# RobotVisionHKA/LiFCal

Hardware: AMD Instinct MI355X
Metric: micro-image obs/sec through Jacobian+Schur at 1M obs (higher is better)
Workload: dtype f64; 1 GPU; metric_web: 334 frames, 24720 points, 999994 micro-image observations, window 10, config 0xf06 (2 radial + tangential, mlCenterAdj, Cauchy(0.5), refine poses+points); lens_selection=reference generator (lifcal_mla_project), obs_per_gpu=999994, n_reduced=2021, deterministic=False

## Files before the change

lifcal_amd/csrc/device_model.hpp:

```cpp
#pragma once
#include <hip/hip_runtime.h>

namespace lifcal {

#define LIFCAL_DEV __device__ __forceinline__

constexpr int NCMAX = 9;
constexpr int LENS_STRIDE = 16;
constexpr int FRAME_STRIDE = 16;

struct CamConsts {
  double fL, bL0, B, ifL;
  double craw[2];
  double sp[2], isp[2];
  double D, iD, e, zC0, gamma, beta;
  double de[3], dzC0[3], dgamma[3], dbeta[3];
  double a, da[3];
  double k[2], p[2];
  double chm[NCMAX];
  double loss_b, loss_c;
};

LIFCAL_DEV void cam_prepare(const double* cam, double spx, double spy, double scale, int n_radial, bool tangential,
                            unsigned fixed_mask, double loss_scale, bool fold, CamConsts& c) {
  double sg[3] = {1.0, 1.0, 1.0};
  double th[3];
  for (int i = 0; i < 3; ++i) { th[i] = cam[i]; if (fold && th[i] < 0.0) { th[i] = -th[i]; sg[i] = -1.0; } }
  c.fL = th[0]; c.bL0 = th[1]; c.B = th[2]; c.ifL = 1.0 / c.fL;
  double dcr[2];
  for (int i = 0; i < 2; ++i) {
    double v = (cam[3 + i] + 0.5) * scale - 0.5; dcr[i] = scale;
    if (fold && v < 0.0) { v = -v; dcr[i] = -scale; }
    c.craw[i] = v;
  }
  c.sp[0] = spx / scale; c.sp[1] = spy / scale; c.isp[0] = 1.0 / c.sp[0]; c.isp[1] = 1.0 / c.sp[1];
  const double D = c.fL - c.bL0, iD = 1.0 / D, iD2 = iD * iD;
  c.D = D; c.iD = iD;
  c.e = c.fL * iD; c.zC0 = c.fL * c.bL0 * iD; c.gamma = c.fL * c.B * iD; c.beta = c.B * iD;
  c.de[0] = -c.bL0 * iD2;          c.de[1] = c.fL * iD2;           c.de[2] = 0.0;
  c.dzC0[0] = -c.bL0 * c.bL0 * iD2; c.dzC0[1] = c.fL * c.fL * iD2;   c.dzC0[2] = 0.0;
  c.dgamma[0] = -c.B * c.bL0 * iD2; c.dgamma[1] = c.fL * c.B * iD2;  c.dgamma[2] = c.fL * iD;
  c.dbeta[0] = -c.B * iD2;          c.dbeta[1] = c.B * iD2;          c.dbeta[2] = iD;
  const double s = c.bL0 + c.B, is = 1.0 / s;
  c.a = c.bL0 * is; c.da[0] = 0.0; c.da[1] = c.B * is * is; c.da[2] = -c.bL0 * is * is;
  c.k[0] = n_radial > 0 ? cam[5] : 0.0; c.k[1] = n_radial > 1 ? cam[6] : 0.0;
  c.p[0] = tangential ? cam[5 + n_radial] : 0.0; c.p[1] = tangential ? cam[6 + n_radial] : 0.0;
  const int nc = 5 + n_radial + (tangential ? 2 : 0);
  for (int j = 0; j < NCMAX; ++j) {
    double ch = 1.0;
    if (j < 3) ch = sg[j]; else if (j < 5) ch = dcr[j - 3];
    const bool live = (j < nc) && !((fixed_mask >> j) & 1u);
    c.chm[j] = live ? ch : 0.0;
  }
  c.loss_b = loss_scale * loss_scale; c.loss_c = 1.0 / c.loss_b;
}

template <int NR, bool TAN>
struct Distortion {
  double dx, dy, A00, A01, A10, A11, r2, r4;
  LIFCAL_DEV void eval(double x, double y, const CamConsts& c, bool want_jac) {
    r2 = x * x + y * y; r4 = r2 * r2;
    double g = 0.0, gp = 0.0;
    if (NR >= 1) { g = c.k[0] * r2; gp = c.k[0]; }
    if (NR >= 2) { g += c.k[1] * r4; gp += 2.0 * c.k[1] * r2; }
    dx = x * g; dy = y * g;
    if (want_jac) { const double xy2 = 2.0 * x * y * gp; A00 = g + 2.0 * x * x * gp; A01 = xy2; A10 = xy2; A11 = g + 2.0 * y * y * gp; }
    if (TAN) {
      dx += c.p[0] * (r2 + 2.0 * x * x) + 2.0 * c.p[1] * x * y;
      dy += c.p[1] * (r2 + 2.0 * y * y) + 2.0 * c.p[0] * x * y;
      if (want_jac) {
        A00 += 6.0 * c.p[0] * x + 2.0 * c.p[1] * y; A01 += 2.0 * c.p[0] * y + 2.0 * c.p[1] * x;
        A10 += 2.0 * c.p[1] * x + 2.0 * c.p[0] * y; A11 += 6.0 * c.p[1] * y + 2.0 * c.p[0] * x;
      }
    }
  }
  LIFCAL_DEV void explicit_partial(int a, double x, double y, double& ex, double& ey) const {
    ex = 0.0; ey = 0.0;
    if (NR >= 1 && a == 2) { ex = x * r2; ey = y * r2; }
    if (NR >= 2 && a == 3) { ex = x * r4; ey = y * r4; }
    if (TAN && a == 2 + NR) { ex = r2 + 2.0 * x * x; ey = 2.0 * x * y; }
    if (TAN && a == 3 + NR) { ex = 2.0 * x * y; ey = r2 + 2.0 * y * y; }
  }
};

template <int NR, bool TAN>
LIFCAL_DEV void lens_eval(const CamConsts& c, double mx, double my, bool want_tangents, double* out) {
  constexpr int NA = 2 + NR + (TAN ? 2 : 0);
  const double cdx = (mx - c.craw[0]) * c.sp[0], cdy = (my - c.craw[1]) * c.sp[1];
// ... 391 lines not shown
```

lifcal_amd/csrc/kernels.hpp:

```cpp
#pragma once
#include <hip/hip_runtime.h>
#include <stdint.h>

#include <type_traits>

#include "../../include/lifcal_ba.h"
#include "device_model.hpp"
#include "lm_step.hpp"

namespace lifcal {

constexpr uint32_t DET_NF_MAX = 20;
constexpr int SCAL_COST = 0, SCAL_BAD_U = 1, SCAL_GMAX0 = 2, SCAL_N = 2 + 64;
constexpr int ST_GTD = 0, ST_DDD = 1, ST_STEP2 = 2, ST_X2 = 3, ST_CAND_COST = 4, ST_CHOL_FAIL = 5, ST_GMAX_RED = 6, ST_DIR = 7, ST_N = 8;

struct TileSet { uint32_t n_tiles; const uint32_t *tile_row0, *slot_pt, *slot_fr, *slot_cnt, *ell_lens; const double *ell_u, *ell_v; };

struct Dev {
  uint32_t F, P, Q, NA, bw, nc, n_tiles, n_slots, n_lenses, n_red, ld, M_local, n_owned;
  uint32_t n_radial, tangential, adj, robust, use_poses, use_points, rank, world;
  uint32_t fixed_mask;
  double spx, spy, scale, loss_scale;
  double lm_min, lm_max;
  double *cam, *views, *pts, *cam_c, *views_c, *pts_c;
// ... 238 lines not shown
      const uint32_t pr = 6 * fr;
      double* Sd = d.Sband + (size_t)fr * (d.bw + 1) * 36;
      const double fm = d.frame_live[fr] != 0 ? 1.0 : 0.0;
#pragma unroll
      for (int a = 0; a < 6; ++a)
#pragma unroll
        for (int bb = 0; bb <= a; ++bb) {
          double v;
          if (a < 3) v = GAG[a][bb]; else if (bb < 3) v = AG[a - 3][bb]; else v = Am[a - 3][bb - 3];
          v *= fm;
          atomicAdd(Sd + a * 6 + bb, v);
          if (a == bb) atomicAdd(d.hdiag + pr + a, v);
        }
#pragma unroll
      for (int a = 0; a < 3; ++a) {
        atomicAdd(d.gB + pr + a, fm * (Gr[0][a] * b[0] + Gr[1][a] * b[1] + Gr[2][a] * b[2]));
        atomicAdd(d.gB + pr + 3 + a, fm * b[a]);
      }
      const uint32_t camrow = 3 * d.Q;
#pragma unroll
      for (int j = 0; j < NC; ++j) {
        double* row = d.Sarrow + (size_t)(camrow + j) * d.ld + pr;
#pragma unroll
        for (int cidx = 0; cidx < 3; ++cidx) atomicAdd(row + cidx, fm * (C[0][j] * Gr[0][cidx] + C[1][j] * Gr[1][cidx] + C[2][j] * Gr[2][cidx]));
#pragma unroll
        for (int cidx = 0; cidx < 3; ++cidx) atomicAdd(row + 3 + cidx, fm * C[cidx][j]);
      }
      if (d.use_points) {
        double AR[3][3], U[3][3], gP[3], Wc[3][NC], Wv[3][6];
#pragma unroll
        for (int i = 0; i < 3; ++i)
#pragma unroll
          for (int j = 0; j < 3; ++j) AR[i][j] = Am[i][0] * R[j] + Am[i][1] * R[3 + j] + Am[i][2] * R[6 + j];
#pragma unroll
        for (int i = 0; i < 3; ++i) {
#pragma unroll
          for (int j = 0; j < 3; ++j) U[i][j] = R[i] * AR[0][j] + R[3 + i] * AR[1][j] + R[6 + i] * AR[2][j];
          gP[i] = R[i] * b[0] + R[3 + i] * b[1] + R[6 + i] * b[2];
#pragma unroll
          for (int j = 0; j < NC; ++j) Wc[i][j] = R[i] * C[0][j] + R[3 + i] * C[1][j] + R[6 + i] * C[2][j];
#pragma unroll
          for (int j = 0; j < 3; ++j) Wv[i][j] = R[i] * AG[0][j] + R[3 + i] * AG[1][j] + R[6 + i] * AG[2][j];
#pragma unroll
          for (int j = 0; j < 3; ++j) Wv[i][3 + j] = R[i] * Am[0][j] + R[3 + i] * Am[1][j] + R[6 + i] * Am[2][j];
        }
        double* acc = d.ptacc + (size_t)pt * 36;
        atomicAdd(acc + 0, U[0][0]); atomicAdd(acc + 1, U[1][0]); atomicAdd(acc + 2, U[2][0]);
        atomicAdd(acc + 3, U[1][1]); atomicAdd(acc + 4, U[2][1]); atomicAdd(acc + 5, U[2][2]);
#pragma unroll
        for (int i = 0; i < 3; ++i) atomicAdd(acc + 6 + i, gP[i]);
#pragma unroll
        for (int i = 0; i < 3; ++i)
#pragma unroll
          for (int j = 0; j < NC; ++j) atomicAdd(acc + 9 + i * NCMAX + j, Wc[i][j]);
        double* wv = d.Wv + (size_t)d.slot_gid[slot] * 18;
#pragma unroll
        for (int i = 0; i < 3; ++i)
#pragma unroll
          for (int j = 0; j < 6; ++j) wv[i * 6 + j] = fm * Wv[i][j];
      }
    }
  }
  const uint32_t camrow = 3 * d.Q, camcol = 6 * d.F + 3 * d.Q;
  {
    int t = 0;
#pragma unroll
    for (int i = 0; i < NC; ++i) {
#pragma unroll
      for (int j = 0; j <= i; ++j) {
        const double s = wave_sum(cc[t]);
        if (lane == (uint32_t)(t & 63)) { atomicAdd(d.Sarrow + (size_t)(camrow + i) * d.ld + camcol + j, s); if (i == j) atomicAdd(d.hdiag + camcol + i, s); }
        ++t;
      }
    }
#pragma unroll
    for (int i = 0; i < NC; ++i) { const double s = wave_sum(gc[i]); if (lane == (uint32_t)i) atomicAdd(d.gB + camcol + i, s); }
    const double s = wave_sum(cost);
    if (lane == 63) atomicAdd(d.scal + SCAL_COST, s);
  }
  if (d.deterministic) det_turn_pass(d, 0, wave);
}

LIFCAL_DEV double finalize_column(const Dev& d, uint32_t t, double radius) {
  const uint32_t F6 = 6 * d.F;
  bool live;
  if (t < F6) live = d.use_poses && d.frame_live[t / 6];
  else if (t < F6 + 3 * d.Q) live = true;
  else live = d.camc->chm[t - F6 - 3 * d.Q] != 0.0;
  double* diag = s_addr(d, t, t);
  double* rhs = d.Sarrow + (size_t)d.NA * d.ld;
  if (live) {
    const double s = d.sig_red[t];
    const double lam = fmin(fmax(d.hdiag[t] * s * s, d.lm_min), d.lm_max) / (lm_radius(d, radius) * s * s);
    d.lam_red[t] = lam;
    *diag += lam;
    rhs[t] = -d.gB[t] + d.rhsacc[t];
  } else {
    d.lam_red[t] = 0.0;
    *diag = 1.0;
    rhs[t] = 0.0;
  }
  return fabs(d.gB[t]);
}

}
#include "sweep2.hpp"
#include "sweep3.hpp"
#include "sweep4.hpp"
namespace lifcal {

__global__ void k_constraints(Dev d, int cost_only, const double* pts, double* cost_out) {
  for (uint32_t t = blockIdx.x * blockDim.x + threadIdx.x; t < d.M_local; t += gridDim.x * blockDim.x) {
  const uint32_t c = d.my_cons[t];
  const uint32_t pi = d.c_i[c], pj = d.c_j[c];
  const double* Pi = pts + 3 * (size_t)pi; const double* Pj = pts + 3 * (size_t)pj;
  const double dx = Pi[0] - Pj[0], dy = Pi[1] - Pj[1], dz = Pi[2] - Pj[2];
  const double n = sqrt(dx * dx + dy * dy + dz * dz);
  const double is = 1.0 / (d.c_sigma[c] + 0.000001);
  const double r = (n - d.c_dist[c]) * is;
  atomicAdd(cost_out, 0.5 * r * r);
  if (cost_only) continue;
  const double in = is / n;
  const double Ji[3] = {dx * in, dy * in, dz * in};
  const uint32_t F6 = 6 * d.F;
  const int32_t qi = d.promoted[pi], qj = d.promoted[pj];
  const uint32_t cj = F6 + 3 * (uint32_t)qj;
  for (int a = 0; a < 3; ++a) {
    for (int b = 0; b <= a; ++b) s_add(d, cj + a, cj + b, Ji[a] * Ji[b]);
    atomicAdd(d.hdiag + cj + a, Ji[a] * Ji[a]);
    atomicAdd(d.gB + cj + a, -Ji[a] * r);
  }
  if (qi < 0) {
    double* acc = d.ptacc + (size_t)pi * 36;
    atomicAdd(acc + 0, Ji[0] * Ji[0]); atomicAdd(acc + 1, Ji[1] * Ji[0]); atomicAdd(acc + 2, Ji[2] * Ji[0]);
    atomicAdd(acc + 3, Ji[1] * Ji[1]); atomicAdd(acc + 4, Ji[2] * Ji[1]); atomicAdd(acc + 5, Ji[2] * Ji[2]);
    for (int a = 0; a < 3; ++a) atomicAdd(acc + 6 + a, Ji[a] * r);
    double* wp = d.Wpart + (size_t)c * 9;
    for (int a = 0; a < 3; ++a) for (int b = 0; b < 3; ++b) wp[a * 3 + b] = -Ji[a] * Ji[b];
  } else {
    const uint32_t ci = F6 + 3 * (uint32_t)qi;
    for (int a = 0; a < 3; ++a) {
      for (int b = 0; b <= a; ++b) s_add(d, ci + a, ci + b, Ji[a] * Ji[b]);
      atomicAdd(d.hdiag + ci + a, Ji[a] * Ji[a]);
      atomicAdd(d.gB + ci + a, Ji[a] * r);
      for (int b = 0; b < 3; ++b) {
        const double v = -Ji[a] * Ji[b];
        if (ci > cj) atomicAdd(s_addr(d, ci + a, cj + b), v); else atomicAdd(s_addr(d, cj + b, ci + a), v);
      }
    }
  }
  }
}

__global__ void k_promote_diag(Dev d) {
  const uint32_t q = blockIdx.x * blockDim.x + threadIdx.x;
  if (q >= d.Q) return;
  const uint32_t p = d.promoted_ids[q];
  const double* acc = d.ptacc + (size_t)p * 36;
  const uint32_t col = 6 * d.F + 3 * q;
  atomicAdd(d.hdiag + col + 0, acc[0]); atomicAdd(d.hdiag + col + 1, acc[3]); atomicAdd(d.hdiag + col + 2, acc[5]);
}

__global__ void k_jacobi(Dev d, int enabled) {
  const uint32_t t = blockIdx.x * blockDim.x + threadIdx.x;
  if (t < d.n_red) d.sig_red[t] = enabled ? 1.0 / (1.0 + sqrt(d.hdiag[t])) : 1.0;
  if (t < d.P) {
    const double* acc = d.ptacc + (size_t)t * 36;
    d.sigP[3 * (size_t)t + 0] = enabled ? 1.0 / (1.0 + sqrt(acc[0])) : 1.0;
    d.sigP[3 * (size_t)t + 1] = enabled ? 1.0 / (1.0 + sqrt(acc[3])) : 1.0;
    d.sigP[3 * (size_t)t + 2] = enabled ? 1.0 / (1.0 + sqrt(acc[5])) : 1.0;
  }
}

struct WBlock { const double* W; uint32_t width, ldw, base; };

LIFCAL_DEV WBlock point_block(const Dev& d, uint32_t p, uint32_t bidx, uint32_t ns) {
  WBlock b;
  if (bidx == 0) { b.W = d.ptacc + (size_t)p * 36 + 9; b.width = d.nc; b.ldw = NCMAX; b.base = 6 * d.F + 3 * d.Q; }
  else if (bidx <= ns) { const uint32_t s = d.pt_slot0[p] + bidx - 1; b.W = d.Wv + (size_t)s * 18; b.width = 6; b.ldw = 6; b.base = 6 * d.gid_fr[s]; }
  else { const uint32_t c = d.pt_cons_list[d.pt_cons0[p] + (bidx - ns - 1)]; b.W = d.Wpart + (size_t)c * 9; b.width = 3; b.ldw = 3; b.base = 6 * d.F + 3 * (uint32_t)d.promoted[d.c_j[c]]; }
  return b;
}

__global__ __launch_bounds__(256) void k_schur(Dev d, double radius) {
  const uint32_t lane = threadIdx.x & 63u;
// ... 181 lines not shown
  double sum = 0.0;
  double* dst = nullptr;
  if (t < n1) {
    if (mode != 0) return;
    const uint32_t f = (uint32_t)(t / BS), r = (uint32_t)(t % BS), dd = r / 36, e = r % 36;
    if (dd > f || (dd == 0 && (e % 6) > (e / 6))) return;
    uint32_t b0, b1; covering(f - dd, f, b0, b1);
    for (uint32_t b = b0; b < b1; ++b) {
      const uint32_t flo = d.blk_flo[b], nf = d.blk_nf[b];
      if (f >= flo + nf) continue;
      const uint32_t lf = f - flo, lj = f - dd - flo;
      sum += d.det_slab[(size_t)b * d.det_stride + (size_t)(lf * (lf + 1) / 2 + lj) * 36 + e];
    }
    dst = d.Sband + t;
  } else if (t < n2) {
    if (mode != 0) return;
    const uint32_t q = (uint32_t)(t - n1), j = q / F6, col = q % F6, f = col / 6;
    uint32_t b0, b1; covering(f, f, b0, b1);
    for (uint32_t b = b0; b < b1; ++b) {
      const uint32_t flo = d.blk_flo[b], nf = d.blk_nf[b];
      if (f >= flo + nf) continue;
      sum += d.det_slab[(size_t)b * d.det_stride + lay.off_cp + (size_t)j * 6 * NFm + 6 * (f - flo) + col % 6];
    }
    dst = d.Sarrow + (size_t)(camrow + j) * d.ld + col;
  } else if (t < n3) {
    if (mode != 0) return;
    return;
  } else if (t < n4) {
    const uint32_t q = (uint32_t)(t - n3), w = q / F6, col = q % F6, f = col / 6;
    if (mode != 0 && w != 1) return;
    uint32_t b0, b1; covering(f, f, b0, b1);
    for (uint32_t b = b0; b < b1; ++b) {
      const uint32_t flo = d.blk_flo[b], nf = d.blk_nf[b];
      if (f >= flo + nf) continue;
      sum += d.det_slab[(size_t)b * d.det_stride + lay.off_vec + (size_t)w * vlen + 6 * (f - flo) + col % 6];
    }
    dst = (w == 0 ? d.gB : (w == 1 ? d.hdiag : d.rhsacc)) + col;
  } else if (t < n5) {
    return;
  } else {
    return;
  }
  *dst += sum;
}

__global__ __launch_bounds__(64) void k_det_reduce_all(Dev d, int mode) {
  const V2Lds lay(d.v2_nfmax, true, 256);
  const uint32_t NFm = lay.nfm, vlen = 6 * NFm + NCMAX + 3, NC = d.nc, NCC = NC * (NC + 1) / 2, nB = d.n_blocks;
  const uint32_t e = blockIdx.x, lane = threadIdx.x;
  const uint32_t camrow = 3 * d.Q, camcol = 6 * d.F + 3 * d.Q;
  uint32_t off; double* dst; bool is_max = false;
  if (e < NCC) {
    if (mode != 0) return;
    uint32_t i = 0; while ((i + 1) * (i + 2) / 2 <= e) ++i;
    off = lay.off_cc + e; dst = d.Sarrow + (size_t)(camrow + i) * d.ld + camcol + (e - i * (i + 1) / 2);
  } else if (e < NCC + 3 * NC) {
    const uint32_t q = e - NCC, w = q / NC, j = q % NC;
    if (mode != 0 && w != 1) return;
    off = lay.off_vec + w * vlen + 6 * NFm + j; dst = (w == 0 ? d.gB : (w == 1 ? d.hdiag : d.rhsacc)) + camcol + j;
  } else {
    if (mode != 0) return;
    const uint32_t q = e - NCC - 3 * NC;
    off = lay.off_fr + q; is_max = q == 2;
    dst = d.scal + (q == 0 ? SCAL_COST : (q == 1 ? SCAL_BAD_U : SCAL_GMAX0 + d.rank));
  }
  double v = 0.0;
  for (uint32_t b = lane; b < nB; b += 64) { const double x = d.det_slab[(size_t)b * d.det_stride + off]; v = is_max ? fmax(v, x) : v + x; }
#pragma unroll
  for (int m = 32; m >= 1; m >>= 1) { const double o = __shfl_xor(v, m, 64); v = is_max ? fmax(v, o) : v + o; }
  if (lane == 0) { if (is_max) *dst = fmax(*dst, v); else *dst += v; }
}

__global__ void k_det_sum(const double* slots, uint32_t n_wg, uint32_t K, double* dst) {
  const uint32_t k = threadIdx.x;
  if (k >= K) return;
  double s = 0.0;
  for (uint32_t g = 0; g < n_wg; ++g) s += slots[(size_t)g * K + k];
  dst[k] += s;
}

constexpr uint32_t FIN_ZERO_PER_WG = 256 * 4;
__global__ void k_finalize(Dev d, double radius, uint32_t n_fin, double* zero, uint32_t n_zero) {
  if (blockIdx.x >= n_fin) {
    const uint32_t n_threads = (gridDim.x - n_fin) * blockDim.x;
    for (uint32_t i = (blockIdx.x - n_fin) * blockDim.x + threadIdx.x; i < n_zero; i += n_threads) zero[i] = 0.0;
    return;
  }
  const uint32_t t = blockIdx.x * blockDim.x + threadIdx.x;
  if (t == 0) d.lm[LM_T0] = (double)__builtin_amdgcn_s_memrealtime();
  double g = 0.0;
  if (t < d.n_red) g = finalize_column(d, t, radius);
#pragma unroll
  for (int m = 32; m >= 1; m >>= 1) g = fmax(g, __shfl_xor(g, m, 64));
  if ((threadIdx.x & 63u) == 0) atomicMax((unsigned long long*)(d.step + ST_GMAX_RED), (unsigned long long)__double_as_longlong(g));
}

__global__ __launch_bounds__(1024) void k_band_chol(Dev d) {
  extern __shared__ __attribute__((aligned(16))) double smem[];
  double* Ld = smem; double* Li = smem + 36; double* failp = smem + 72;
  double* panel = d.panel_g ? d.panel_g : smem + 80;
  const uint32_t tid = threadIdx.x, nt = blockDim.x;
  const uint32_t F = d.F, bw = d.bw, NAx = d.NA + 1, ld = d.ld;
  if (tid == 0) *failp = 0.0;
  __syncthreads();
  for (uint32_t j = 0; j < F; ++j) {
    double* Sjj = d.Sband + (size_t)j * (bw + 1) * 36;
    if (tid == 0) {
      double L[6][6];
      for (int a = 0; a < 6; ++a) for (int b = 0; b <= a; ++b) L[a][b] = Sjj[a * 6 + b];
      bool ok = true;
      for (int c = 0; c < 6; ++c) {
        double dg = L[c][c];
        for (int k = 0; k < c; ++k) dg -= L[c][k] * L[c][k];
        if (!(dg > 0.0)) { ok = false; dg = 1.0; }
        dg = sqrt(dg); L[c][c] = dg;
        for (int r = c + 1; r < 6; ++r) { double s = L[r][c]; for (int k = 0; k < c; ++k) s -= L[r][k] * L[c][k]; L[r][c] = s / dg; }
      }
      if (!ok) *failp = 1.0;
      double I[6][6];
      for (int c = 0; c < 6; ++c) {
        for (int r = 0; r < 6; ++r) I[r][c] = 0.0;
        I[c][c] = 1.0 / L[c][c];
        for (int r = c + 1; r < 6; ++r) { double s = 0.0; for (int k = c; k < r; ++k) s -= L[r][k] * I[k][c]; I[r][c] = s / L[r][r]; }
      }
      for (int a = 0; a < 6; ++a) for (int b = 0; b < 6; ++b) { Ld[a * 6 + b] = (b <= a) ? L[a][b] : 0.0; Li[a * 6 + b] = (b <= a) ? I[a][b] : 0.0; }
      for (int a = 0; a < 6; ++a) for (int b = 0; b <= a; ++b) Sjj[a * 6 + b] = L[a][b];
      for (int k = 0; k < 36; ++k) d.Linv[(size_t)j * 36 + k] = Li[k];
    }
    __syncthreads();
    const uint32_t nbel = min(bw, F - 1 - j);
    const uint32_t nrows = 6 * nbel + NAx;
    for (uint32_t r = tid; r < nrows; r += nt) {
      double* src;
      if (r < 6 * nbel) { const uint32_t i = j + 1 + r / 6; src = d.Sband + ((size_t)i * (bw + 1) + (i - j)) * 36 + (r % 6) * 6; }
      else src = d.Sarrow + (size_t)(r - 6 * nbel) * ld + 6 * j;
      double x[6], y[6];
#pragma unroll
      for (int k = 0; k < 6; ++k) x[k] = src[k];
#pragma unroll
      for (int c = 0; c < 6; ++c) { double s = 0.0;
#pragma unroll
        for (int k = 0; k <= c; ++k) s += x[k] * Li[c * 6 + k];
        y[c] = s; }
#pragma unroll
      for (int k = 0; k < 6; ++k) { src[k] = y[k]; panel[(size_t)r * 6 + k] = y[k]; }
    }
    __syncthreads();
    const uint32_t nb6 = 6 * nbel;
    const uint64_t nband = (uint64_t)nb6 * (nb6 + 1) / 2;
    const uint64_t narrow = (uint64_t)NAx * nb6;
    const uint64_t naa = (uint64_t)NAx * (NAx + 1) / 2;
    for (uint64_t t = tid; t < nband + narrow + naa; t += nt) {
      uint32_t r, cidx; double* dst;
      if (t < nband) {
        r = (uint32_t)((sqrt(8.0 * (double)t + 1.0) - 1.0) * 0.5);
        while ((uint64_t)r * (r + 1) / 2 > t) --r;
        while ((uint64_t)(r + 1) * (r + 2) / 2 <= t) ++r;
        cidx = (uint32_t)(t - (uint64_t)r * (r + 1) / 2);
        const uint32_t bi = j + 1 + r / 6, bc = j + 1 + cidx / 6;
        dst = d.Sband + ((size_t)bi * (bw + 1) + (bi - bc)) * 36 + (r % 6) * 6 + (cidx % 6);
      } else if (t < nband + narrow) {
        const uint64_t u = t - nband; const uint32_t a = (uint32_t)(u / nb6); cidx = (uint32_t)(u % nb6); r = nb6 + a;
        dst = d.Sarrow + (size_t)a * ld + 6 * (j + 1) + cidx;
      } else {
        const uint64_t u = t - nband - narrow;
        uint32_t a = (uint32_t)((sqrt(8.0 * (double)u + 1.0) - 1.0) * 0.5);
        while ((uint64_t)a * (a + 1) / 2 > u) --a;
        while ((uint64_t)(a + 1) * (a + 2) / 2 <= u) ++a;
// ... 451 lines not shown
```

lifcal_amd/csrc/sweep3.hpp:

```cpp
#pragma once

namespace lifcal {

template <int NR, bool TAN, bool ADJ, int WR, class ET = double>
__global__ __launch_bounds__(128 * WR, 2) void k_sweep3(Dev d, double radius, int mode) {
  constexpr bool F32 = sizeof(ET) == 4;
  constexpr int NC = 5 + NR + (TAN ? 2 : 0);
  constexpr int NCC = NC * (NC + 1) / 2;
  constexpr int HV = 6 + 2 * NC + 2;
  constexpr uint32_t LP = 64u * WR;
  constexpr uint32_t NT = 2u * LP;
  static_assert(HV * LP <= V2Lds::zd_for(LP), "hand-off buffer must fit the Z matrix");
  if (radius < 0.0 && d.lm[LM_TERMINATION] != 0.0) return;
  extern __shared__ __attribute__((aligned(16))) double sm[];
  const V2Lds lay(d.v2_nfmax, true, LP);
  const uint32_t NFm = lay.nfm, vlen = 6 * NFm + NCMAX + 3;
  double* Spp = sm; double* Scp = sm + lay.off_cp; double* Scc = sm + lay.off_cc;
  double* vgB = sm + lay.off_vec; double* vhd = vgB + vlen; double* vrhs = vhd + vlen;
  double* Fr = sm + lay.off_fr;
  double* slab = sm + lay.off_slab;
  double* Zd = sm + lay.off_zd;
  double* misc = sm + lay.off_misc;
  uint32_t* pidl = (uint32_t*)(misc + MISC_DOUBLES);
  unsigned short* colinfo = (unsigned short*)(misc + MISC_DOUBLES + 32);
  uint32_t flip = 0;
#ifndef LIFCAL_NO_ROLE_FLIP
  if (WR == 2) flip = (__builtin_amdgcn_s_getreg(6 | (0 << 6) | (7 << 11)) != 0) ? LP : 0u;
#endif
  const uint32_t tid = threadIdx.x ^ flip, lane = tid & 63u, w = tid >> 6;
  const bool role_b = w >= (uint32_t)WR;
  const uint32_t wl = w & (uint32_t)(WR - 1);
  const uint32_t t256 = tid & (LP - 1u);
  const uint32_t b = blockIdx.x;
  const uint32_t flo = d.blk_flo[b], nf = d.blk_nf[b];
  const uint32_t ncol = 6 * nf + NC + 1, ncolp = (ncol + 15u) & ~15u;
  const uint32_t zs = ncolp + 2;
  const CamConsts c = *d.camc;
#ifdef LIFCAL_STAMPS
  unsigned long long st_acc[16] = {0, 0, 0, 0, 0, 0, 0, 0, 0, 0, 0, 0, 0, 0, 0, 0}, st_last = 0;
  if (tid == 0 || tid == LP) { asm volatile("s_memtime %0\n\ts_waitcnt lgkmcnt(0)" : "=s"(st_last) :: "memory"); }
#define STAMPB(i) do { if (tid == LP) { unsigned long long t_; asm volatile("s_memtime %0\n\ts_waitcnt lgkmcnt(0)" : "=s"(t_) :: "memory"); st_acc[i] += t_ - st_last; st_last = t_; } } while (0)
#else
#define STAMPB(i) do { } while (0)
#endif
  const uint32_t ps_begin = d.blk_pass0[b], ps_end = d.blk_pass0[b + 1];
  uint32_t nx_np = 0, nx_gid0 = 0, nx_si = 0, nx_pt = 0, nx_fp = 0, nx_gid = 0, nx_r[2] = {0, 0};
  uint32_t vz;
  asm volatile("v_mov_b32 %0, 0" : "=v"(vz));
  auto fetch_pass = [&](uint32_t q) {
    nx_np = d.pass_np[q + vz]; nx_gid0 = d.pass_gid0[q + vz];
    nx_si = d.v2_slot[(size_t)q * LP + t256]; nx_pt = d.v2f_pt[(size_t)q * LP + t256]; nx_gid = d.v2_gidx[(size_t)q * LP + t256];
    nx_r[0] = d.v2_tile_row0[q * WR + wl + vz]; nx_r[1] = d.v2_tile_row0[q * WR + wl + 1 + vz];
    nx_fp = d.v2_passpt[(size_t)q * 64 + (tid & 63u)];
  };
  if (ps_begin < ps_end) fetch_pass(ps_begin);
  { double2* z2 = reinterpret_cast<double2*>(sm); for (uint32_t i = tid; i < lay.off_slab / 2; i += NT) z2[i] = double2{0.0, 0.0}; }
  if (tid == 0 && (lay.off_slab & 1u)) sm[lay.off_slab - 1] = 0.0;
  if (tid < MISC_DOUBLES) misc[tid] = 0.0;
  for (uint32_t cI = tid; cI < ncolp; cI += NT)
    colinfo[cI] = (cI < 6 * nf) ? (unsigned short)(((cI / 6) << 8) | (cI % 6)) : (cI < ncol - 1 ? (unsigned short)(0x8000u | (cI - 6 * nf)) : (unsigned short)0xC000u);

  auto zero_slab = [&]() { for (uint32_t i = tid; i < lay.np_max * SLAB_STRIDE; i += NT) slab[i] = 0.0; };
  auto zero_zd = [&](uint32_t krows) { double2* z2 = reinterpret_cast<double2*>(Zd); for (uint32_t i = tid; i < (krows * zs) / 2; i += NT) z2[i] = double2{0.0, 0.0}; };
  auto z_phase = [&](uint32_t np) {
    const uint32_t nwc = ncol - 1;
    const uint32_t nth = NT / nwc > 0 ? NT / nwc : 1;
    const uint32_t gi = tid / nwc, cidx = tid - gi * nwc;
    if (gi < nth || nwc > NT) {
      for (uint32_t cc0 = cidx; cc0 < nwc; cc0 += (nwc > NT ? NT : nwc * nth)) {
#pragma unroll 4
        for (uint32_t lp = (nwc > NT ? 0 : gi); lp < np; lp += (nwc > NT ? 1 : nth)) {
          const double* acc = slab + lp * SLAB_STRIDE;
          double* z = Zd + (size_t)(3 * lp) * zs + cc0;
          const double w0 = z[0], w1 = z[zs], w2 = z[2 * zs];
          if (cc0 >= 6 * nf) {
            double* ga = d.ptacc + (size_t)pidl[lp] * 36 + 9 + (cc0 - 6 * nf);
            ga[0] = w0; ga[NCMAX] = w1; ga[2 * NCMAX] = w2;
          }
          z[0] = acc[0] * w0; z[zs] = acc[1] * w0 + acc[3] * w1; z[2 * zs] = acc[2] * w0 + acc[4] * w1 + acc[5] * w2;
        }
      }
    }
  };
  struct LaneGeom { double R[9], Y[3], Gr[3][3]; };
  auto lane_geom = [&](uint32_t fr, uint32_t pt, LaneGeom& q) {
    const double* ft = d.ft + (size_t)fr * FRAME_STRIDE;
    const double* P = d.pts + 3 * (size_t)pt;
#pragma unroll
    for (int k = 0; k < 9; ++k) q.R[k] = ft[k];
    const double P0 = P[0], P1 = P[1], P2 = P[2];
#pragma unroll
    for (int k = 0; k < 3; ++k) q.Y[k] = q.R[3 * k] * P0 + q.R[3 * k + 1] * P1 + q.R[3 * k + 2] * P2;
    const double c0 = ft[12], s0 = ft[13], n0 = q.R[2], n1 = q.R[5], n2 = q.R[8];
    q.Gr[0][0] = 0.0;     q.Gr[0][1] = c0 * q.Y[2] - s0 * q.Y[1]; q.Gr[0][2] = n1 * q.Y[2] - n2 * q.Y[1];
    q.Gr[1][0] = -q.Y[2]; q.Gr[1][1] = s0 * q.Y[0];               q.Gr[1][2] = n2 * q.Y[0] - n0 * q.Y[2];
    q.Gr[2][0] = q.Y[1];  q.Gr[2][1] = -c0 * q.Y[0];              q.Gr[2][2] = n0 * q.Y[1] - n1 * q.Y[0];
  };
  const uint32_t frs = NFm * lay.nrep;
  struct RunMask { double m1, m2, m4, m8; bool head; };
  auto run_masks = [&](uint32_t cnt, uint32_t lf) {
    const int key = cnt > 0 ? (int)lf : (int)(0x7F000000u + lane);
    RunMask r;
    r.m1 = __builtin_amdgcn_update_dpp(-1, key, 0x101, 0xf, 0xf, false) == key ? 1.0 : 0.0;
    r.m2 = __builtin_amdgcn_update_dpp(-1, key, 0x102, 0xf, 0xf, false) == key ? 1.0 : 0.0;
    r.m4 = __builtin_amdgcn_update_dpp(-1, key, 0x104, 0xf, 0xf, false) == key ? 1.0 : 0.0;
    r.m8 = __builtin_amdgcn_update_dpp(-1, key, 0x108, 0xf, 0xf, false) == key ? 1.0 : 0.0;
    r.head = cnt > 0 && __builtin_amdgcn_update_dpp(-1, key, 0x111, 0xf, 0xf, false) != key;
    return r;
  };
  auto run_sum = [](double v, const RunMask& r) {
    auto shl = [](double x, auto ctrl) {
      const int lo = __double2loint(x), hi = __double2hiint(x);
      return __hiloint2double(__builtin_amdgcn_update_dpp(0, hi, decltype(ctrl)::value, 0xf, 0xf, true),
                              __builtin_amdgcn_update_dpp(0, lo, decltype(ctrl)::value, 0xf, 0xf, true));
    };
    v = fma(shl(v, std::integral_constant<int, 0x101>{}), r.m1, v);
    v = fma(shl(v, std::integral_constant<int, 0x102>{}), r.m2, v);
    v = fma(shl(v, std::integral_constant<int, 0x104>{}), r.m4, v);
    v = fma(shl(v, std::integral_constant<int, 0x108>{}), r.m8, v);
    return v;
  };
  uint32_t* hw_written = (uint32_t*)(misc + 4) + wl;
  uint32_t* hw_read = (uint32_t*)(misc + 4) + 4 + wl;
  uint32_t* eval_done = (uint32_t*)(misc + 3);
  const bool det = d.deterministic != 0;
  uint32_t* turn = (uint32_t*)(misc + 8) + (role_b ? 1 : 0);
  uint32_t my_turn = wl;
  auto wait_for = [](uint32_t* flag, uint32_t need) {
    while (__hip_atomic_load(flag, __ATOMIC_ACQUIRE, __HIP_MEMORY_SCOPE_WORKGROUP) < need) __builtin_amdgcn_s_sleep(2);
  };
  auto publish = [](uint32_t* flag, uint32_t value) {
    asm volatile("s_waitcnt lgkmcnt(0)" ::: "memory");
    __hip_atomic_store(flag, value, __ATOMIC_RELEASE, __HIP_MEMORY_SCOPE_WORKGROUP);
  };

  const uint32_t nmt = (ncol + 3u) >> 2, ntri = nmt * (nmt + 1) / 2;
  auto tri_decode = [](uint32_t t, uint32_t& mi, uint32_t& mj) {
    mi = (uint32_t)((sqrtf(8.0f * (float)t + 1.0f) - 1.0f) * 0.5f);
    while (mi * (mi + 1) / 2 > t) --mi;
    while ((mi + 1) * (mi + 2) / 2 <= t) ++mi;
    mj = t - mi * (mi + 1) / 2;
  };
  auto gemm_tile = [&](uint32_t mi, uint32_t mj, uint32_t kfirst, uint32_t kstep, uint32_t krows, double (&acc16)[4][4]) {
    const double* za = Zd + 4 * mi;
    const double* zb = Zd + 4 * mj;
    double2 cur[4][4];
#pragma unroll
    for (int r = 0; r < 4; ++r) {
      cur[r][0] = *reinterpret_cast<const double2*>(za + (size_t)(kfirst + r) * zs);
      cur[r][1] = *reinterpret_cast<const double2*>(za + (size_t)(kfirst + r) * zs + 2);
      cur[r][2] = *reinterpret_cast<const double2*>(zb + (size_t)(kfirst + r) * zs);
      cur[r][3] = *reinterpret_cast<const double2*>(zb + (size_t)(kfirst + r) * zs + 2);
    }
#pragma unroll 2
    for (uint32_t k0 = kfirst; k0 < krows; k0 += kstep) {
      double2 nxt[4][4];
      const uint32_t kn = (k0 + kstep < krows) ? k0 + kstep : k0;
#pragma unroll
      for (int r = 0; r < 4; ++r) {
        nxt[r][0] = *reinterpret_cast<const double2*>(za + (size_t)(kn + r) * zs);
// ... 132 lines not shown
#pragma unroll
          for (int a = 0; a < 2; ++a) {
            const double q0 = Jq[a][0], q1 = Jq[a][1], q2 = Jq[a][2], ra = r[a];
            A[0] += q0 * q0; A[1] += q0 * q1; A[2] += q0 * q2;
            A[3] += q1 * q1; A[4] += q1 * q2; A[5] += q2 * q2;
            bv[0] += q0 * ra; bv[1] += q1 * ra; bv[2] += q2 * ra;
          }
        }
        {
          const ET* Lp = lens_tab + (size_t)ln * LENS_STRIDE;
#pragma unroll
          for (int i = 0; i < LENS_STRIDE; ++i) Ln[i] = Lp[i];
          if constexpr (F32) { wn0 = d.ltw[2 * (size_t)ln]; wn1 = d.ltw[2 * (size_t)ln + 1]; }
          const uint32_t kk = (k + 2 < kmax) ? k + 2 : kmax - 1;
          const size_t at = ((size_t)row0 + kk) * 64 + lane;
          uc = obs_u[at]; vc = obs_v[at]; lc = d.v2_lens[at];
        }
        publish(hw_written, hbase + k + 1);
      };
      for (uint32_t k = 0; k < kmax; k += 2) {
        step(k, ua, va, la, lb);
        if (k + 1 < kmax) step(k + 1, ub, vb, lb, la);
      }
      hbase += kmax;
      LaneGeom q;
      { uint32_t fr2 = fr, pt2 = pt; asm volatile("" : "+v"(fr2), "+v"(pt2)); lane_geom(fr2, pt2, q); }
      asm volatile("" :: "v"(nx_si), "v"(nx_pt), "v"(nx_fp), "v"(nx_np), "v"(nx_gid0), "v"(nx_gid), "v"(nx_r[0]), "v"(nx_r[1]));
      asm volatile("" :: "v"(fsg0), "v"(fsg1), "v"(fsg2));
      STAMP(7);
      lds_barrier();
      if (mode == 0) zero_zd(krows);
      lds_barrier();
      if (det) wait_for(turn, my_turn);
      if (cnt > 0) {
        const double Am[3][3] = {{A[0], A[1], A[2]}, {A[1], A[3], A[4]}, {A[2], A[4], A[5]}};
        const double (&R)[9] = q.R; const double (&Gr)[3][3] = q.Gr;
        double AG[3][3], GAG[3][3];
#pragma unroll
        for (int i = 0; i < 3; ++i)
#pragma unroll
          for (int j = 0; j < 3; ++j) AG[i][j] = Am[i][0] * Gr[0][j] + Am[i][1] * Gr[1][j] + Am[i][2] * Gr[2][j];
#pragma unroll
        for (int i = 0; i < 3; ++i)
#pragma unroll
          for (int j = 0; j < 3; ++j) GAG[i][j] = Gr[0][i] * AG[0][j] + Gr[1][i] * AG[1][j] + Gr[2][i] * AG[2][j];
        RunMask rm = run_masks(cnt, lf);
        const bool fpose = d.frame_live[fr] != 0;
        rm.head = rm.head && fpose;
        double* fr_acc = Fr + lf;
        {
          int vi = 0;
#pragma unroll
          for (int a = 0; a < 6; ++a)
#pragma unroll
            for (int bb = 0; bb <= a; ++bb) {
              double v;
              if (a < 3) v = GAG[a][bb]; else if (bb < 3) v = AG[a - 3][bb]; else v = Am[a - 3][bb - 3];
              v = run_sum(v, rm);
              if (rm.head) atomicAdd(fr_acc + (size_t)vi * frs, v);
              ++vi;
            }
#pragma unroll
          for (int a = 0; a < 3; ++a) { const double v = run_sum(Gr[0][a] * bv[0] + Gr[1][a] * bv[1] + Gr[2][a] * bv[2], rm); if (rm.head) atomicAdd(fr_acc + (size_t)(21 + a) * frs, v); }
#pragma unroll
          for (int a = 0; a < 3; ++a) { const double v = run_sum(bv[a], rm); if (rm.head) atomicAdd(fr_acc + (size_t)(24 + a) * frs, v); }
        }
        double AR[3][3];
#pragma unroll
        for (int i = 0; i < 3; ++i)
#pragma unroll
          for (int j = 0; j < 3; ++j) AR[i][j] = Am[i][0] * R[j] + Am[i][1] * R[3 + j] + Am[i][2] * R[6 + j];
        double* acc = slab + lp * SLAB_STRIDE;
#pragma unroll
        for (int i = 0; i < 3; ++i) {
#pragma unroll
          for (int j = 0; j <= i; ++j) {
            const double u_ij = R[i] * AR[0][j] + R[3 + i] * AR[1][j] + R[6 + i] * AR[2][j];
            const int pos = (i == 0) ? 0 : (i == 1 ? (j == 0 ? 1 : 3) : (j == 0 ? 2 : (j == 1 ? 4 : 5)));
            atomicAdd(acc + pos, u_ij);
          }
        }
        if (mode == 0) {
          { double* ga = d.Av + (size_t)gidx * 6;
#pragma unroll
            for (int k = 0; k < 6; ++k) ga[k] = A[k]; }
#pragma unroll
          for (int i = 0; i < 3; ++i) {
            atomicAdd(acc + 6 + i, R[i] * bv[0] + R[3 + i] * bv[1] + R[6 + i] * bv[2]);
            double* zrow = Zd + (size_t)(3 * lp + i) * zs + 6 * lf;
            double w6[6];
#pragma unroll
            for (int j = 0; j < 3; ++j) { w6[j] = R[i] * AG[0][j] + R[3 + i] * AG[1][j] + R[6 + i] * AG[2][j]; w6[3 + j] = R[i] * Am[0][j] + R[3 + i] * Am[1][j] + R[6 + i] * Am[2][j]; }
            const bool rot = (lp & 1u) != 0;
#pragma unroll
            for (int jj = 0; jj < 6; ++jj) {
              const double wv = rot ? w6[(jj + 1) % 6] : w6[jj];
              const uint32_t col = rot ? (uint32_t)((jj + 1) % 6) : (uint32_t)jj;
              if (fpose) atomicAdd(zrow + col, wv);
            }
          }
        }
      }
      if (det) { publish(turn, my_turn + 1); my_turn += (uint32_t)WR; }
      STAMP(6);
      asm volatile("s_waitcnt lgkmcnt(0)" ::: "memory");
      if (lane == 0) __hip_atomic_fetch_add(eval_done, 1u, __ATOMIC_RELAXED, __HIP_MEMORY_SCOPE_WORKGROUP);
      ++passes_done;
      if (w == 0) wait_for(eval_done, (uint32_t)WR * passes_done);
      STAMP(1);
      if (tid < np) {
        const uint32_t p = fp;
        pidl[tid] = p;
        double* acc = slab + tid * SLAB_STRIDE;
        double U0 = acc[0], U1 = acc[1], U2 = acc[2], U3 = acc[3], U4 = acc[4], U5 = acc[5];
        if (mode == 1) {
          double* ga = d.ptacc + (size_t)p * 36;
          ga[0] = U0; ga[3] = U3; ga[5] = U5;
        } else {
          const double g0 = acc[6], g1 = acc[7], g2 = acc[8];
          double lam[3];
          {
            const double h[3] = {U0, U3, U5}, sgv[3] = {fsg0, fsg1, fsg2};
#pragma unroll
            for (int k = 0; k < 3; ++k) { const double sg = sgv[k]; lam[k] = fmin(fmax(h[k] * sg * sg, d.lm_min), d.lm_max) / (lm_radius(d, radius) * sg * sg); }
          }
          U0 += lam[0]; U3 += lam[1]; U5 += lam[2];
          bool ok = U0 > 0.0;
          double i00 = rsqrt(U0);
          const double l10 = U1 * i00, l20 = U2 * i00;
          const double d11 = U3 - l10 * l10; ok = ok && (d11 > 0.0);
          double i11 = rsqrt(d11);
          const double l21 = (U4 - l20 * l10) * i11;
          const double d22 = U5 - l20 * l20 - l21 * l21; ok = ok && (d22 > 0.0);
          double i22 = rsqrt(d22);
          double m10 = -l10 * i00 * i11, m21 = -l21 * i11 * i22, m20 = -(l20 * i00 + l21 * m10) * i22;
          if (!ok) { i00 = i11 = i22 = m10 = m21 = m20 = 0.0; atomicAdd(misc + 1, 1.0); }
          double* gu = d.Uinv + 9 * (size_t)p;
          const double v00 = i00 * i00 + m10 * m10 + m20 * m20, v01 = m10 * i11 + m20 * m21, v02 = m20 * i22;
          const double v11 = i11 * i11 + m21 * m21, v12 = m21 * i22, v22 = i22 * i22;
          gu[0] = v00; gu[1] = v01; gu[2] = v02; gu[3] = v01; gu[4] = v11; gu[5] = v12; gu[6] = v02; gu[7] = v12; gu[8] = v22;
          double* gl = d.lamP + 3 * (size_t)p; gl[0] = lam[0]; gl[1] = lam[1]; gl[2] = lam[2];
          double* ga = d.ptacc + (size_t)p * 36;
          ga[6] = g0; ga[7] = g1; ga[8] = g2;
          const double gm = fmax(fabs(g0), fmax(fabs(g1), fabs(g2)));
          atomicMax((unsigned long long*)(misc + 2), (unsigned long long)__double_as_longlong(gm));
          acc[0] = i00; acc[1] = m10; acc[2] = m20; acc[3] = i11; acc[4] = m21; acc[5] = i22;
          double* z0 = Zd + (size_t)(3 * tid) * zs + (ncol - 1);
          z0[0] = i00 * g0; z0[zs] = m10 * g0 + i11 * g1; z0[2 * zs] = m20 * g0 + m21 * g1 + i22 * g2;
        }
      }
      lds_barrier();
      STAMP(2);
      if (mode == 0) {
        z_phase(np);
        lds_barrier();
        STAMP(3);
        if (keep_tiles) {
          if (tid < ntri) gemm_tile(mi0, mj0, 0, ksplit ? 8u : 4u, krows, tacc);
        } else {
          for (uint32_t t = tid; t < ntri; t += (share_tiles ? NT : LP)) {
            uint32_t mi, mj; tri_decode(t, mi, mj);
            double acc16[4][4];
#pragma unroll
            for (int i = 0; i < 4; ++i)
#pragma unroll
              for (int j = 0; j < 4; ++j) acc16[i][j] = 0.0;
            gemm_tile(mi, mj, 0, 4, krows, acc16);
            emit_tile(mi, mj, acc16);
          }
        }
      }
      lds_barrier();
      STAMP(4);
    }
    STAMP(8);
    if (keep_tiles && tid < ntri) {
      if (ksplit) {
#pragma unroll
        for (int i = 0; i < 4; ++i)
#pragma unroll
          for (int j = 0; j < 4; ++j) tacc[i][j] += bt[(i * 4 + j) * LP + tid];
      }
      uint32_t ci4[4], cj4[4];
#pragma unroll
      for (int i = 0; i < 4; ++i) { const uint32_t ci = 4 * mi0 + i, cj = 4 * mj0 + i; ci4[i] = colinfo[ci < ncolp ? ci : 0]; cj4[i] = colinfo[cj < ncolp ? cj : 0]; }
      uint32_t off[4][4]; double sg[4][4];
      const uint32_t dummy = lay.off_zd + 1024u + tid;
#pragma unroll
      for (int i = 0; i < 4; ++i)
#pragma unroll
        for (int j = 0; j < 4; ++j) {
          const uint32_t ci = 4 * mi0 + i, cj = 4 * mj0 + j, ii = ci4[i], jj = cj4[j];
          uint32_t o = dummy; double sgn = -1.0;
          if (!(ci >= ncol || cj >= ncol || ci < cj)) {
            if (!(ii & 0x8000u)) {
              const uint32_t lfi = ii >> 8, lfj = jj >> 8;
              o = (lfi * (lfi + 1) / 2 + lfj) * 36 + (ii & 0xFFu) * 6 + (jj & 0xFFu);
            } else if (!(ii & 0x4000u)) {
              const uint32_t jc = ii & 0xFFu;
              o = !(jj & 0x8000u) ? lay.off_cp + jc * 6 * NFm + cj : lay.off_cc + jc * (jc + 1) / 2 + (jj & 0xFFu);
            } else if (cj < ncol - 1) {
              o = lay.off_vec + 2 * vlen + (!(jj & 0x8000u) ? cj : 6 * NFm + (jj & 0xFFu));
              sgn = 1.0;
            }
          }
          off[i][j] = o; sg[i][j] = sgn;
        }
      double oldv[4][4];
#pragma unroll
      for (int i = 0; i < 4; ++i)
#pragma unroll
        for (int j = 0; j < 4; ++j) oldv[i][j] = sm[off[i][j]];
#pragma unroll
      for (int i = 0; i < 4; ++i)
#pragma unroll
        for (int j = 0; j < 4; ++j) sm[off[i][j]] = oldv[i][j] + sg[i][j] * tacc[i][j];
    }
    STAMP(9);
    if (d.robust) cost += 0.5 * c.loss_b * (log(lmant) + (double)lexp * 0.6931471805599453);
    cost = wave_sum_dpp(cost);
    if (det) wait_for(turn, my_turn);
    if (lane == 63) atomicAdd(misc + 0, cost);
    if (det) publish(turn, my_turn + 1);
    lds_barrier(); lds_barrier();
  } else {
    double cc[NCC], gc[NC];
// ... 83 lines not shown
#pragma unroll
          for (int j = 0; j < NC; ++j) wc[j] = R[i] * C[0][j] + R[3 + i] * C[1][j] + R[6 + i] * C[2][j];
          const bool rot = (lp & 1u) != 0;
#pragma unroll
          for (int jj = 0; jj < NC; ++jj) atomicAdd(zrow + (rot ? (uint32_t)((jj + 1) % NC) : (uint32_t)jj), rot ? wc[(jj + 1) % NC] : wc[jj]);
        }
      }
      if (det) { publish(turn, my_turn + 1); my_turn += (uint32_t)WR; }
      STAMPB(3);
      lds_barrier();
      STAMPB(4);
      if (mode == 0) {
        z_phase(np);
        lds_barrier();
      }
      if (ksplit && t256 < ntri) {
        uint32_t mi, mj; tri_decode(t256, mi, mj);
        double acc16[4][4];
#pragma unroll
        for (int i = 0; i < 4; ++i)
#pragma unroll
          for (int j = 0; j < 4; ++j) acc16[i][j] = bt[(i * 4 + j) * LP + t256];
        gemm_tile(mi, mj, 4, 8, krows, acc16);
#pragma unroll
        for (int i = 0; i < 4; ++i)
#pragma unroll
          for (int j = 0; j < 4; ++j) bt[(i * 4 + j) * LP + t256] = acc16[i][j];
      }
      if (share_tiles) {
        for (uint32_t t = tid; t < ntri; t += NT) {
          uint32_t mi, mj; tri_decode(t, mi, mj);
          double acc16[4][4];
#pragma unroll
          for (int i = 0; i < 4; ++i)
#pragma unroll
            for (int j = 0; j < 4; ++j) acc16[i][j] = 0.0;
          gemm_tile(mi, mj, 0, 4, krows, acc16);
          emit_tile(mi, mj, acc16);
        }
      }
      lds_barrier();
      STAMPB(5);
    }
    {
      int t = 0;
#pragma unroll
      for (int i = 0; i < NC; ++i) {
        gc[i] *= c.chm[i];
#pragma unroll
        for (int j = 0; j <= i; ++j) cc[t++] *= c.chm[i] * c.chm[j];
      }
    }
    constexpr int NVB = NCC + NC;
    constexpr uint32_t NROWS = 4u * WR;
    {
      double* red = Zd;
      const uint32_t rowi = t256 >> 4;
      const bool tail = (lane & 15u) == 15u;
#pragma unroll
      for (int idx = 0; idx < NVB; ++idx) {
        double v = (idx < NCC) ? cc[idx < NCC ? idx : 0] : gc[(idx - NCC) >= 0 && (idx - NCC) < NC ? idx - NCC : 0];
        v = dpp_add_step<0x111, 0xf>(v); v = dpp_add_step<0x112, 0xf>(v); v = dpp_add_step<0x114, 0xf>(v); v = dpp_add_step<0x118, 0xf>(v);
        if (tail) red[rowi * NVB + idx] = v;
      }
      lds_barrier();
      if (t256 < (uint32_t)NVB) {
        const int idx = (int)t256;
        double sacc = 0.0;
#pragma unroll
        for (uint32_t k = 0; k < NROWS; ++k) sacc += red[k * NVB + idx];
        if (idx < NCC) {
          int i = 0; while ((i + 1) * (i + 2) / 2 <= idx) ++i;
          if (mode == 0) Scc[idx] += sacc;
          if (idx == i * (i + 1) / 2 + i) vhd[6 * NFm + i] += sacc;
        } else {
          vgB[6 * NFm + (idx - NCC)] += sacc;
        }
      }
      lds_barrier();
    }
  }
  lds_barrier();
  STAMP(10);
  for (uint32_t i = tid; i < FRV * nf; i += NT) {
    const uint32_t v = i / nf, lf = i % nf;
    double sacc = 0.0;
    for (uint32_t r = 0; r < lay.nrep; ++r) sacc += Fr[(size_t)v * NFm * lay.nrep + r * NFm + lf];
    if (v < 21) {
      uint32_t a = 0; while ((a + 1) * (a + 2) / 2 <= v) ++a;
      const uint32_t bb = v - a * (a + 1) / 2;
      Spp[(size_t)(lf * (lf + 1) / 2 + lf) * 36 + a * 6 + bb] += sacc;
      if (a == bb) vhd[6 * lf + a] += sacc;
    } else if (v < 27) {
      vgB[6 * lf + (v - 21)] += sacc;
    } else if (mode == 0 && v < 27 + 6 * (uint32_t)NC) {
      const uint32_t j = (v - 27) / 6, ci = (v - 27) % 6;
      Scp[(size_t)j * 6 * NFm + 6 * lf + ci] += sacc;
    }
  }
  lds_barrier();
  STAMP(11);
  if (det) {
    double* out = d.det_slab + (size_t)b * d.det_stride;
    for (uint32_t i = tid; i < lay.off_fr; i += NT) out[i] = sm[i];
    if (tid < 3) out[lay.off_fr + tid] = misc[tid];
    return;
  }
  const uint32_t F6 = 6 * d.F, camrow = 3 * d.Q, camcol = F6 + 3 * d.Q;
  for (uint32_t i = tid; i < 6 * nf; i += NT) atomicAdd(d.hdiag + 6 * flo + i, vhd[i]);
  if (tid < (uint32_t)NC) atomicAdd(d.hdiag + camcol + tid, vhd[6 * NFm + tid]);
  if (mode == 0) {
    const uint32_t npp = nf * (nf + 1) / 2;
    for (uint32_t i = tid; i < npp * 36; i += NT) {
      const uint32_t blk = i / 36, e = i % 36;
      uint32_t a = (uint32_t)((sqrtf(8.0f * (float)blk + 1.0f) - 1.0f) * 0.5f);
      while (a * (a + 1) / 2 > blk) --a;
      while ((a + 1) * (a + 2) / 2 <= blk) ++a;
      const uint32_t bb = blk - a * (a + 1) / 2, dd = a - bb;
      const double v = Spp[i];
      if (dd <= d.bw && v != 0.0 && !(dd == 0 && (e % 6) > (e / 6))) atomicAdd(d.Sband + ((size_t)(flo + a) * (d.bw + 1) + dd) * 36 + e, v);
    }
    for (uint32_t i = tid; i < (uint32_t)NC * 6 * nf; i += NT) {
      const uint32_t j = i / (6 * nf), cidx = i % (6 * nf);
      atomicAdd(d.Sarrow + (size_t)(camrow + j) * d.ld + 6 * flo + cidx, Scp[(size_t)j * 6 * NFm + cidx]);
    }
    if (tid < (uint32_t)NCC) {
      uint32_t i = 0; while ((i + 1) * (i + 2) / 2 <= tid) ++i;
      const uint32_t j = tid - i * (i + 1) / 2;
      atomicAdd(d.Sarrow + (size_t)(camrow + i) * d.ld + camcol + j, Scc[tid]);
    }
    for (uint32_t i = tid; i < 6 * nf; i += NT) { atomicAdd(d.gB + 6 * flo + i, vgB[i]); atomicAdd(d.rhsacc + 6 * flo + i, vrhs[i]); }
    if (tid < (uint32_t)NC) { atomicAdd(d.gB + camcol + tid, vgB[6 * NFm + tid]); atomicAdd(d.rhsacc + camcol + tid, vrhs[6 * NFm + tid]); }
    if (tid == 0) {
      atomicAdd(d.scal + SCAL_COST, misc[0]);
      if (misc[1] != 0.0) atomicAdd(d.scal + SCAL_BAD_U, misc[1]);
      atomicMax((unsigned long long*)(d.scal + SCAL_GMAX0 + d.rank), *(unsigned long long*)(misc + 2));
    }
  }
#ifdef LIFCAL_STAMPS
  lds_barrier();
  STAMP(5);
  if ((tid == 0 || tid == LP) && d.dbg) for (int i = 0; i < 16; ++i) d.dbg[(size_t)b * 32 + (tid == 0 ? 0 : 16) + i] = st_acc[i];
#endif
}

}
```

Measured before the change: 9.248 billion obs/s.

## Use streaming stores, vectorize zeroing, branchless finalize, reorder global atomics

Adds inline-asm global stores with the sc1 cache-policy bit for per-point and per-observation outputs in sweep3 (ptacc, Av, Uinv, lamP). The zero-fill in k_finalize now writes double2 with head/tail handling, and finalize_column issues all loads up front and selects live/dead results without branching. Camera-block and scalar atomics in sweep3 are moved earlier, before the frame-reduction loop, and the remaining atomic loops are reordered. Together these aim to cut cache pollution, store-instruction count and atomic tail latency. The hand-written asm with s_nop bypasses compiler scheduling and may add stalls.

```diff
diff --git a/lifcal_amd/csrc/device_model.hpp b/lifcal_amd/csrc/device_model.hpp
--- a/lifcal_amd/csrc/device_model.hpp
+++ b/lifcal_amd/csrc/device_model.hpp
@@ -4,6 +4,15 @@
 namespace lifcal {
 
 #define LIFCAL_DEV __device__ __forceinline__
+
+typedef double stream_d2 __attribute__((ext_vector_type(2)));
+LIFCAL_DEV void store_stream(double* p, double v) {
+  asm volatile("global_store_dwordx2 %0, %1, off sc1\n\ts_nop 1" :: "v"(p), "v"(v) : "memory");
+}
+LIFCAL_DEV void store_stream(double* p, double v0, double v1) {
+  const stream_d2 v{v0, v1};
+  asm volatile("global_store_dwordx4 %0, %1, off sc1\n\ts_nop 1" :: "v"(p), "v"(v) : "memory");
+}
 
 constexpr int NCMAX = 9;
 constexpr int LENS_STRIDE = 16;
diff --git a/lifcal_amd/csrc/kernels.hpp b/lifcal_amd/csrc/kernels.hpp
--- a/lifcal_amd/csrc/kernels.hpp
+++ b/lifcal_amd/csrc/kernels.hpp
@@ -344,25 +344,19 @@
 }
 
 LIFCAL_DEV double finalize_column(const Dev& d, uint32_t t, double radius) {
-  const uint32_t F6 = 6 * d.F;
-  bool live;
-  if (t < F6) live = d.use_poses && d.frame_live[t / 6];
-  else if (t < F6 + 3 * d.Q) live = true;
-  else live = d.camc->chm[t - F6 - 3 * d.Q] != 0.0;
+  const uint32_t F6 = 6 * d.F, A0 = F6 + 3 * d.Q;
   double* diag = s_addr(d, t, t);
   double* rhs = d.Sarrow + (size_t)d.NA * d.ld;
-  if (live) {
-    const double s = d.sig_red[t];
-    const double lam = fmin(fmax(d.hdiag[t] * s * s, d.lm_min), d.lm_max) / (lm_radius(d, radius) * s * s);
-    d.lam_red[t] = lam;
-    *diag += lam;
-    rhs[t] = -d.gB[t] + d.rhsacc[t];
-  } else {
-    d.lam_red[t] = 0.0;
-    *diag = 1.0;
-    rhs[t] = 0.0;
-  }
-  return fabs(d.gB[t]);
+  const uint32_t fl = t < F6 ? (uint32_t)d.frame_live[t / 6] : 1u;
+  const double ch = t >= A0 ? d.camc->chm[t - A0] : 1.0;
+  const double s = d.sig_red[t], h = d.hdiag[t], g = d.gB[t], ra = d.rhsacc[t], dg = *diag;
+  const double rad = lm_radius(d, radius);
+  const bool live = t < F6 ? (d.use_poses && fl) : ch != 0.0;
+  const double lam = live ? fmin(fmax(h * s * s, d.lm_min), d.lm_max) / (rad * s * s) : 0.0;
+  d.lam_red[t] = lam;
+  *diag = live ? dg + lam : 1.0;
+  rhs[t] = live ? -g + ra : 0.0;
+  return fabs(g);
 }
 
 }
@@ -710,8 +704,13 @@
 constexpr uint32_t FIN_ZERO_PER_WG = 256 * 4;
 __global__ void k_finalize(Dev d, double radius, uint32_t n_fin, double* zero, uint32_t n_zero) {
   if (blockIdx.x >= n_fin) {
-    const uint32_t n_threads = (gridDim.x - n_fin) * blockDim.x;
-    for (uint32_t i = (blockIdx.x - n_fin) * blockDim.x + threadIdx.x; i < n_zero; i += n_threads) zero[i] = 0.0;
+    const uint32_t n_threads = (gridDim.x - n_fin) * blockDim.x, t0 = (blockIdx.x - n_fin) * blockDim.x + threadIdx.x;
+    const uint32_t odd = (uint32_t)(((uintptr_t)zero >> 3) & 1u), head = odd < n_zero ? odd : n_zero;
+    const uint32_t n2 = (n_zero - head) / 2;
+    double2* z2 = reinterpret_cast<double2*>(zero + head);
+    for (uint32_t i = t0; i < n2; i += n_threads) z2[i] = double2{0.0, 0.0};
+    if (t0 == 0 && head) zero[0] = 0.0;
+    if (t0 == 0 && head + 2 * n2 < n_zero) zero[n_zero - 1] = 0.0;
     return;
   }
   const uint32_t t = blockIdx.x * blockDim.x + threadIdx.x;
diff --git a/lifcal_amd/csrc/sweep3.hpp b/lifcal_amd/csrc/sweep3.hpp
--- a/lifcal_amd/csrc/sweep3.hpp
+++ b/lifcal_amd/csrc/sweep3.hpp
@@ -75,7 +75,7 @@
           const double w0 = z[0], w1 = z[zs], w2 = z[2 * zs];
           if (cc0 >= 6 * nf) {
             double* ga = d.ptacc + (size_t)pidl[lp] * 36 + 9 + (cc0 - 6 * nf);
-            ga[0] = w0; ga[NCMAX] = w1; ga[2 * NCMAX] = w2;
+            store_stream(ga, w0); store_stream(ga + NCMAX, w1); store_stream(ga + 2 * NCMAX, w2);
           }
           z[0] = acc[0] * w0; z[zs] = acc[1] * w0 + acc[3] * w1; z[2 * zs] = acc[2] * w0 + acc[4] * w1 + acc[5] * w2;
         }
@@ -374,8 +374,7 @@
         }
         if (mode == 0) {
           { double* ga = d.Av + (size_t)gidx * 6;
-#pragma unroll
-            for (int k = 0; k < 6; ++k) ga[k] = A[k]; }
+            store_stream(ga, A[0], A[1]); store_stream(ga + 2, A[2], A[3]); store_stream(ga + 4, A[4], A[5]); }
 #pragma unroll
           for (int i = 0; i < 3; ++i) {
             atomicAdd(acc + 6 + i, R[i] * bv[0] + R[3 + i] * bv[1] + R[6 + i] * bv[2]);
@@ -407,7 +406,7 @@
         double U0 = acc[0], U1 = acc[1], U2 = acc[2], U3 = acc[3], U4 = acc[4], U5 = acc[5];
         if (mode == 1) {
           double* ga = d.ptacc + (size_t)p * 36;
-          ga[0] = U0; ga[3] = U3; ga[5] = U5;
+          store_stream(ga, U0); store_stream(ga + 3, U3); store_stream(ga + 5, U5);
         } else {
           const double g0 = acc[6], g1 = acc[7], g2 = acc[8];
           double lam[3];
@@ -430,10 +429,16 @@
           double* gu = d.Uinv + 9 * (size_t)p;
           const double v00 = i00 * i00 + m10 * m10 + m20 * m20, v01 = m10 * i11 + m20 * m21, v02 = m20 * i22;
           const double v11 = i11 * i11 + m21 * m21, v12 = m21 * i22, v22 = i22 * i22;
-          gu[0] = v00; gu[1] = v01; gu[2] = v02; gu[3] = v01; gu[4] = v11; gu[5] = v12; gu[6] = v02; gu[7] = v12; gu[8] = v22;
-          double* gl = d.lamP + 3 * (size_t)p; gl[0] = lam[0]; gl[1] = lam[1]; gl[2] = lam[2];
-          double* ga = d.ptacc + (size_t)p * 36;
-          ga[6] = g0; ga[7] = g1; ga[8] = g2;
+          {
+            const double vu[9] = {v00, v01, v02, v01, v11, v12, v02, v12, v22};
+#pragma unroll
+            for (int k = 0; k < 9; ++k) store_stream(gu + k, vu[k]);
+          }
+          double* gl = d.lamP + 3 * (size_t)p;
+          double* ga = d.ptacc + (size_t)p * 36 + 6;
+#pragma unroll
+          for (int k = 0; k < 3; ++k) store_stream(gl + k, lam[k]);
+          store_stream(ga, g0); store_stream(ga + 1, g1); store_stream(ga + 2, g2);
           const double gm = fmax(fabs(g0), fmax(fabs(g1), fabs(g2)));
           atomicMax((unsigned long long*)(misc + 2), (unsigned long long)__double_as_longlong(gm));
           acc[0] = i00; acc[1] = m10; acc[2] = m20; acc[3] = i11; acc[4] = m21; acc[5] = i22;
@@ -683,6 +688,23 @@
   }
   lds_barrier();
   STAMP(10);
+  if (!det) {
+    const uint32_t F6 = 6 * d.F, camrow = 3 * d.Q, camcol = F6 + 3 * d.Q;
+    if (mode == 0 && tid < (uint32_t)NCC) {
+      uint32_t i = 0; while ((i + 1) * (i + 2) / 2 <= tid) ++i;
+      const uint32_t j = tid - i * (i + 1) / 2;
+      atomicAdd(d.Sarrow + (size_t)(camrow + i) * d.ld + camcol + j, Scc[tid]);
+    }
+    if (tid < (uint32_t)NC) {
+      atomicAdd(d.hdiag + camcol + tid, vhd[6 * NFm + tid]);
+      if (mode == 0) { atomicAdd(d.gB + camcol + tid, vgB[6 * NFm + tid]); atomicAdd(d.rhsacc + camcol + tid, vrhs[6 * NFm + tid]); }
+    }
+    if (mode == 0 && tid == 0) {
+      atomicAdd(d.scal + SCAL_COST, misc[0]);
+      if (misc[1] != 0.0) atomicAdd(d.scal + SCAL_BAD_U, misc[1]);
+      atomicMax((unsigned long long*)(d.scal + SCAL_GMAX0 + d.rank), *(unsigned long long*)(misc + 2));
+    }
+  }
   for (uint32_t i = tid; i < FRV * nf; i += NT) {
     const uint32_t v = i / nf, lf = i % nf;
     double sacc = 0.0;
@@ -709,8 +731,12 @@
   }
   const uint32_t F6 = 6 * d.F, camrow = 3 * d.Q, camcol = F6 + 3 * d.Q;
   for (uint32_t i = tid; i < 6 * nf; i += NT) atomicAdd(d.hdiag + 6 * flo + i, vhd[i]);
-  if (tid < (uint32_t)NC) atomicAdd(d.hdiag + camcol + tid, vhd[6 * NFm + tid]);
   if (mode == 0) {
+    for (uint32_t i = tid; i < 6 * nf; i += NT) { atomicAdd(d.gB + 6 * flo + i, vgB[i]); atomicAdd(d.rhsacc + 6 * flo + i, vrhs[i]); }
+    for (uint32_t i = tid; i < (uint32_t)NC * 6 * nf; i += NT) {
+      const uint32_t j = i / (6 * nf), cidx = i % (6 * nf);
+      atomicAdd(d.Sarrow + (size_t)(camrow + j) * d.ld + 6 * flo + cidx, Scp[(size_t)j * 6 * NFm + cidx]);
+    }
     const uint32_t npp = nf * (nf + 1) / 2;
     for (uint32_t i = tid; i < npp * 36; i += NT) {
       const uint32_t blk = i / 36, e = i % 36;
@@ -721,22 +747,6 @@
       const double v = Spp[i];
       if (dd <= d.bw && v != 0.0 && !(dd == 0 && (e % 6) > (e / 6))) atomicAdd(d.Sband + ((size_t)(flo + a) * (d.bw + 1) + dd) * 36 + e, v);
     }
-    for (uint32_t i = tid; i < (uint32_t)NC * 6 * nf; i += NT) {
-      const uint32_t j = i / (6 * nf), cidx = i % (6 * nf);
-      atomicAdd(d.Sarrow + (size_t)(camrow + j) * d.ld + 6 * flo + cidx, Scp[(size_t)j * 6 * NFm + cidx]);
-    }
-    if (tid < (uint32_t)NCC) {
-      uint32_t i = 0; while ((i + 1) * (i + 2) / 2 <= tid) ++i;
-      const uint32_t j = tid - i * (i + 1) / 2;
-      atomicAdd(d.Sarrow + (size_t)(camrow + i) * d.ld + camcol + j, Scc[tid]);
-    }
-    for (uint32_t i = tid; i < 6 * nf; i += NT) { atomicAdd(d.gB + 6 * flo + i, vgB[i]); atomicAdd(d.rhsacc + 6 * flo + i, vrhs[i]); }
-    if (tid < (uint32_t)NC) { atomicAdd(d.gB + camcol + tid, vgB[6 * NFm + tid]); atomicAdd(d.rhsacc + camcol + tid, vrhs[6 * NFm + tid]); }
-    if (tid == 0) {
-      atomicAdd(d.scal + SCAL_COST, misc[0]);
-      if (misc[1] != 0.0) atomicAdd(d.scal + SCAL_BAD_U, misc[1]);
-      atomicMax((unsigned long long*)(d.scal + SCAL_GMAX0 + d.rank), *(unsigned long long*)(misc + 2));
-    }
   }
 #ifdef LIFCAL_STAMPS
   lds_barrier();
```

Result: faster. 9.608 billion obs/s, median of 6 (+3.9%).
